# nguyenduchuyiu/marl-delivery

Hardware: AMD Instinct MI355X
Metric: agent-steps/sec (whole node), map1 5-agent 4096 envs, 1/2/4/8 MI355X (higher is better)
Workload: dtype int32+fp64

## Files before the change

marl-delivery_amd/csrc/mdl_device.hpp:

```cpp
#pragma once
#include <hip/hip_runtime.h>
#include <stdint.h>

#if !defined(MDL_PROFILING_BUILD) && \
    (defined(MDL_EXP_NOWAIT) || defined(MDL_EXP_NOTUPLES) || defined(MDL_EXP_NOLDS) || defined(MDL_ABLATE) || \
     defined(MDL_STAMPS))
#error "MDL_EXP_NOWAIT / MDL_EXP_NOTUPLES / MDL_EXP_NOLDS / MDL_ABLATE / MDL_STAMPS need -DMDL_PROFILING_BUILD"
#endif
#ifndef MDL_ABLATE
#define MDL_ABLATE 0
#endif

namespace mdl {

constexpr int WAVE = 64;
constexpr int MT_N = 624;
constexpr int MT_M = 397;
constexpr int MAX_MAPS = 8;
constexpr int PKG_PAD = 256;

enum : int { ST_NONE = 0, ST_WAITING = 1, ST_IN_TRANSIT = 2, ST_DELIVERED = 3 };
enum : int { MV_S = 0, MV_L = 1, MV_R = 2, MV_U = 3, MV_D = 4, MV_OTHER = 5 };
enum : int { SH_PICK = 0, SH_ONTIME, SH_LATE, SH_CLOSER, SH_WPICK, SH_WDROP, SH_STUCK, SH_IDLE, SH_AWAY };

struct MapDesc {
    int H, W, nfree;
    int grid_off;
    int free_off;
    int rank_off;
    float inv_hw;
    int bits_off;
    int mvc_off;
};

struct __align__(16) EnvScalars {
    int32_t t;
    uint32_t ctr;
    double total;
};
enum : uint32_t { RT_MOVE = 1u, RT_ONTIME = 2u, RT_LATE = 4u };

enum : uint32_t { PS_STATUS = 3u, PS_PRESENT = 4u, PS_TRANSIT = 8u, PS_SURVIVOR = 16u, PS_FLAGS = 31u };
constexpr int PS_RANK_SHIFT = 5;

constexpr uint32_t ORD_EPISODE = 0x400u;

struct DevParams {
    int E, A, P, T;
    double move_cost, delivery_reward, delay_reward;
    double cost_sum[9];
    float shaping[9];
    int stale;
    int obsT, MO, MP, MR, MPs;
    int n_maps;
    int key32_dsh;
    MapDesc maps[MAX_MAPS];
    const uint8_t* grids;
    const uint8_t* movevalid;
    const uint8_t* movevalid_cell;
    const uint32_t* gridbits;
    const uint16_t* free_cells;
    const uint16_t* rank;
    const uint8_t* env_map;
    uint32_t* rob;
    uint64_t* pkg;
    uint16_t* pstate;
    EnvScalars* es;
    uint32_t* mt;
    int32_t* mt_pos;
    uint64_t* trk;
    double* ep_total;
    int32_t* ep_len;
    const double* obs_recip;
    int obs_plane_words;
    int obs_small;
    int key7_dsh;
    double cost_fold[65];
};

__host__ __device__ __forceinline__ uint32_t rob_pack(int cell, int carry, uint32_t valid_mask ) {
    return (uint32_t)cell | ((uint32_t)carry << 16) | ((valid_mask & 0x1eu) << 26);
}
__host__ __device__ __forceinline__ int rob_cell(uint32_t w) { return (int)(w & 0xffffu); }
__host__ __device__ __forceinline__ int rob_carry(uint32_t w) { return (int)((w >> 16) & 0x7ffu); }
__host__ __device__ __forceinline__ uint32_t rob_valid(uint32_t w) { return (w >> 26) & 0x1eu; }

__device__ __forceinline__ int lane_id() { return (int)(threadIdx.x & 63); }
__device__ __forceinline__ int wave_id() { return __builtin_amdgcn_readfirstlane((int)(threadIdx.x >> 6)); }

__device__ __forceinline__ int xcd_slot(int b, int nb) { return (b & 7) * (nb >> 3) + min(b & 7, nb & 7) + (b >> 3); }
__device__ __forceinline__ int xcd_block() {
    return xcd_slot((int)blockIdx.x, (int)gridDim.x);
}

__device__ __forceinline__ void wave_sync() {
    __builtin_amdgcn_fence(__ATOMIC_RELEASE, "wavefront");
    __builtin_amdgcn_wave_barrier();
    __builtin_amdgcn_fence(__ATOMIC_ACQUIRE, "wavefront");
}

__device__ __forceinline__ uint64_t ballot(bool p) { return __ballot(p); }

#define GLOBAL __attribute__((address_space(1)))
typedef unsigned int u32x4 __attribute__((ext_vector_type(4)));

template <class T>
__device__ __forceinline__ void pin(T& v) { asm volatile("" : "+s"(v)); }

__device__ __forceinline__ int rdl(int v, int j) { return __builtin_amdgcn_readlane(v, j); }
__device__ __forceinline__ float rdlf(float v, int j) {
    return __int_as_float(__builtin_amdgcn_readlane(__float_as_int(v), j));
}
__device__ __forceinline__ int uni(int v) { return __builtin_amdgcn_readfirstlane(v); }

__device__ __forceinline__ uint32_t lmask(bool b) {
    uint32_t x = b ? ~0u : 0u;
    asm("" : "+v"(x));
    return x;
}
__device__ __forceinline__ uint32_t vbit(uint64_t m, int lane) { return 0u - (uint32_t)((m >> lane) & 1ull); }
__device__ __forceinline__ float fmask(uint32_t m, float a) { return __uint_as_float(m & __float_as_uint(a)); }
__device__ __forceinline__ float fpick(uint32_t m, float a, float b) {
    return __uint_as_float((m & __float_as_uint(a)) | (~m & __float_as_uint(b)));
}
__device__ __forceinline__ int ipick(uint32_t m, int a, int b) { return (int)((m & (uint32_t)a) | (~m & (uint32_t)b)); }

__device__ __forceinline__ int popc64(uint64_t m) { return __popcll(m); }
__device__ __forceinline__ int ffs64(uint64_t m) { return __ffsll((long long)m) - 1; }
__device__ __forceinline__ uint64_t lanemask_lt() {
    int l = lane_id();
    return l == 0 ? 0ull : (~0ull >> (64 - l));
}

__device__ __forceinline__ uint32_t wave_min_u32(uint32_t v) {
    const int id = (int)0xffffffff;
    uint32_t t;
    t = (uint32_t)__builtin_amdgcn_update_dpp(id, (int)v, 0x111, 0xf, 0xf, false); v = t < v ? t : v;
    t = (uint32_t)__builtin_amdgcn_update_dpp(id, (int)v, 0x112, 0xf, 0xf, false); v = t < v ? t : v;
    t = (uint32_t)__builtin_amdgcn_update_dpp(id, (int)v, 0x114, 0xf, 0xf, false); v = t < v ? t : v;
    t = (uint32_t)__builtin_amdgcn_update_dpp(id, (int)v, 0x118, 0xf, 0xf, false); v = t < v ? t : v;
    t = (uint32_t)__builtin_amdgcn_update_dpp(id, (int)v, 0x142, 0xa, 0xf, false); v = t < v ? t : v;
    t = (uint32_t)__builtin_amdgcn_update_dpp(id, (int)v, 0x143, 0xc, 0xf, false); v = t < v ? t : v;
    return (uint32_t)__builtin_amdgcn_readlane((int)v, 63);
}

__device__ __forceinline__ void wave_min_u32x2(uint32_t u, uint32_t v, uint32_t& mu, uint32_t& mv) {
    const int id = (int)0xffffffff;
    uint32_t a, b;
#define MDL_MIN2(ctl, rm)                                                                  \
    a = (uint32_t)__builtin_amdgcn_update_dpp(id, (int)u, ctl, rm, 0xf, false);            \
    b = (uint32_t)__builtin_amdgcn_update_dpp(id, (int)v, ctl, rm, 0xf, false);            \
    u = a < u ? a : u;                                                                     \
    v = b < v ? b : v;
    MDL_MIN2(0x111, 0xf)
    MDL_MIN2(0x112, 0xf)
    MDL_MIN2(0x114, 0xf)
    MDL_MIN2(0x118, 0xf)
    MDL_MIN2(0x142, 0xa)
    MDL_MIN2(0x143, 0xc)
#undef MDL_MIN2
    mu = (uint32_t)__builtin_amdgcn_readlane((int)u, 63);
    mv = (uint32_t)__builtin_amdgcn_readlane((int)v, 63);
}

__device__ __forceinline__ int wave_min8_lane(int a) { return ((a >> 1) << 4) | ((a & 1) << 3); }
__device__ __forceinline__ uint32_t wave_min8_u32(const uint32_t (&k)[8]) {
    uint32_t m[4], n[2];
#pragma unroll
    for (int i = 0; i < 4; i++) {
        const auto r = __builtin_amdgcn_permlane32_swap(k[i], k[i + 4], false, false);
        m[i] = r[0] < r[1] ? r[0] : r[1];
    }
#pragma unroll
    for (int i = 0; i < 2; i++) {
        const auto r = __builtin_amdgcn_permlane16_swap(m[i], m[i + 2], false, false);
        n[i] = r[0] < r[1] ? r[0] : r[1];
    }
    const bool hi = (lane_id() & 8) != 0;
    const uint32_t keep = hi ? n[1] : n[0], send = hi ? n[0] : n[1];
    const int id = (int)0xffffffff;
    uint32_t t = (uint32_t)__builtin_amdgcn_update_dpp(id, (int)send, 0x128, 0xf, 0xf, false);
    uint32_t v = t < keep ? t : keep;
    t = (uint32_t)__builtin_amdgcn_update_dpp(id, (int)v, 0x141, 0xf, 0xf, false);
    v = t < v ? t : v;
    t = (uint32_t)__builtin_amdgcn_update_dpp(id, (int)v, 0x4E, 0xf, 0xf, false);
    v = t < v ? t : v;
    t = (uint32_t)__builtin_amdgcn_update_dpp(id, (int)v, 0xB1, 0xf, 0xf, false);
    return t < v ? t : v;
}

__device__ __forceinline__ float qdiv_r(int a, double y) { return (float)((double)a * y); }

__device__ __forceinline__ float qdiv(int a, int b) { return (float)a / (float)b; }

__device__ __forceinline__ int fdivi(int i, int d, float inv) {
    int q = (int)((float)i * inv);
    int r = i - q * d;
    if (r < 0) q -= 1;
    else if (r >= d) q += 1;
    return q;
}

__device__ __forceinline__ int cell_r(int pc) { return pc & 255; }
__device__ __forceinline__ int cell_c(int pc) { return (pc >> 8) & 255; }
__device__ __forceinline__ int manhattan(int a, int b) {
    return abs(cell_r(a) - cell_r(b)) + abs(cell_c(a) - cell_c(b));
}
__device__ __forceinline__ int manhattan_sad(int a, int b) {
    return (int)__builtin_amdgcn_sad_u8((uint32_t)a, (uint32_t)b, 0u);
}

__device__ __forceinline__ int pk_start(uint64_t v) { return (int)(v & 0xffff); }
__device__ __forceinline__ int pk_target(uint64_t v) { return (int)((v >> 16) & 0xffff); }
__device__ __forceinline__ int pk_st(uint64_t v) { return (int)((v >> 32) & 0xffff); }
__device__ __forceinline__ int pk_dl(uint64_t v) { return (int)(v >> 48); }
__device__ __forceinline__ uint64_t pk_make(int start, int target, int st, int dl) {
    return (uint64_t)(uint32_t)start | ((uint64_t)(uint32_t)target << 16) | ((uint64_t)(uint32_t)st << 32) |
           ((uint64_t)(uint32_t)dl << 48);
}

__device__ __forceinline__ void decode_action(int a, int fmt, int& mv, int& op) {
    if (fmt == 0) {
        const int q = a / 5;
        const int m = a - 5 * q;
        mv = (0x30214 >> (4 * m)) & 0xf;
        op = q >= 3 ? 0 : q;
    } else {
        mv = a & 7;
        op = (a >> 3) & 3;
        if (mv > MV_OTHER) mv = MV_OTHER;
    }
}

__device__ inline void mt_twist(uint32_t* key) {
    const int lane = lane_id();
    for (int base = 0; base < MT_N; base += WAVE) {
        const int i = base + lane;
        uint32_t v = 0;
        if (i < MT_N) {
            const uint32_t y = (key[i] & 0x80000000u) | (key[i + 1 == MT_N ? 0 : i + 1] & 0x7fffffffu);
            const int k = i + MT_M < MT_N ? i + MT_M : i + MT_M - MT_N;
            v = key[k] ^ (y >> 1) ^ ((y & 1u) ? 0x9908b0dfu : 0u);
        }
        wave_sync();
        if (i < MT_N) key[i] = v;
        wave_sync();
    }
}

struct MTState {
    uint32_t* key;
    int pos;
};

__device__ inline uint32_t mt_next32(MTState& s) {
    if (s.pos == MT_N) {
        mt_twist(s.key);
        s.pos = 0;
    }
    uint32_t y = s.key[s.pos];
    s.pos++;
    y ^= (y >> 11);
    y ^= (y << 7) & 0x9d2c5680u;
    y ^= (y << 15) & 0xefc60000u;
    y ^= (y >> 18);
    return (uint32_t)uni((int)y);
}

__device__ inline int randint(MTState& s, int lo, int hi) {
    const uint32_t rng = (uint32_t)(hi - 1 - lo);
    if (rng == 0) return lo;
    uint32_t mask = rng;
    mask |= mask >> 1; mask |= mask >> 2; mask |= mask >> 4; mask |= mask >> 8; mask |= mask >> 16;
    uint32_t v;
    do {
        v = mt_next32(s) & mask;
    } while (v > rng);
    return lo + (int)v;
}

struct ResetOut {
    int robot_cell;
};

__device__ inline int reset_env(MTState& mt, const DevParams& p, const MapDesc& md, uint64_t* pk, uint8_t* pst,
                                uint64_t* scratch, uint16_t* taken) {
    const int lane = lane_id();
    const int A = p.A, P = p.P;
    const uint16_t* fl = p.free_cells + md.free_off;
    const int F = md.nfree;
    int my_cell = 0;
    int ntk = 0;
    for (int i = 0; i < A; i++) {
        const int k = randint(mt, 0, F - i);
        int idx = k;
        for (int q = 0; q < ntk; q++) {
            const int tq = taken[q];
            if (tq <= idx) idx++;
            else break;
        }
        if (lane == 0) {
            int q = ntk;
            while (q > 0 && taken[q - 1] > idx) {
                taken[q] = taken[q - 1];
                q--;
            }
            taken[q] = (uint16_t)idx;
        }
        ntk++;
        wave_sync();
        if (lane == i) my_cell = fl[idx];
    }
    const int N = md.H;
    const int lim = A < 20 ? A : 20;
    for (int i = 0; i < P; i++) {
        const int s_idx = randint(mt, 0, F);
        int t_idx;
        do {
            t_idx = randint(mt, 0, F);
        } while (t_idx == s_idx);
        const int to_dl = 10 + randint(mt, N / 2, 3 * N);
        const int st = (i <= lim) ? 0 : randint(mt, 1, p.T);
        if (lane == 0) scratch[i] = pk_make(s_idx, t_idx, st, st + to_dl);
    }
    wave_sync();
    for (int j = lane; j < P; j += WAVE) {
        const uint64_t v = scratch[j];
        scratch[j] = pk_make(fl[pk_start(v)], fl[pk_target(v)], pk_st(v), pk_dl(v));
    }
    wave_sync();
    for (int j0 = 0; j0 < P; j0 += WAVE) {
        const int j = j0 + lane;
        uint64_t v = 0;
        int sj = 0, rank = 0;
        if (j < P) {
            v = scratch[j];
            sj = pk_st(v);
        }
        for (int i = 0; i < P; i++) {
            const int si = pk_st(scratch[i]);
            rank += (si < sj) || (si == sj && i < j);
        }
        if (j < P) {
            pk[rank] = v;
        }
    }
    wave_sync();
    for (int j = lane; j < P; j += WAVE) pst[j] = pk_st(pk[j]) == 0 ? ST_WAITING : ST_NONE;
    wave_sync();
    return my_cell;
}

struct TrkFresh {
    static constexpr bool kIdIndexed = true;
    const uint64_t* pk;
    const uint8_t* ps;
    int n;
    __device__ int count() const { return n; }
    __device__ bool present(int j) const { const int s = ps[j] & PS_STATUS; return s == ST_WAITING || s == ST_IN_TRANSIT; }
    __device__ bool in_transit(int j) const { return (ps[j] & PS_STATUS) == ST_IN_TRANSIT; }
    __device__ uint64_t data(int j) const { return pk[j]; }
    __device__ int id(int j) const { return j + 1; }
    __device__ uint32_t order(int j) const { return (uint32_t)j; }
    __device__ int slot_of(int id) const { return (id >= 1 && id <= n && present(id - 1)) ? id - 1 : -1; }
};

struct TrkStale {
    static constexpr bool kIdIndexed = true;
    const uint8_t* ps;
    const uint64_t* td;
    const uint32_t* tq;
    int n;
    __device__ int count() const { return n; }
    __device__ bool present(int j) const { return (ps[j] & PS_PRESENT) != 0; }
    __device__ bool in_transit(int j) const { return (ps[j] & PS_TRANSIT) != 0; }
    __device__ uint64_t data(int j) const { return td[j]; }
    __device__ int id(int j) const { return j + 1; }
    __device__ uint32_t order(int j) const { return tq[j]; }
    __device__ int slot_of(int id) const { return (id >= 1 && id <= n && present(id - 1)) ? id - 1 : -1; }
};

struct TrkView {
    static constexpr bool kIdIndexed = false;
    const int32_t* ids;
    const uint8_t* flag;
    const uint64_t* pk;
    int n;
    __device__ int count() const { return n; }
    __device__ bool present(int j) const { return flag[j] & 1; }
    __device__ bool in_transit(int j) const { return (flag[j] & 2) != 0; }
    __device__ uint64_t data(int j) const { return pk[j]; }
    __device__ int id(int j) const { return ids[j]; }
    __device__ uint32_t order(int j) const { return (uint32_t)j; }
    __device__ int slot_of(int id) const {
        for (int j = 0; j < n; j++)
            if (ids[j] == id) return j;
        return -1;
    }
};

template <class Trk>
__device__ inline float shaped_agent(const Trk& trk, const float* C, bool active, int prev_cell, int prev_carry,
                                     int cur_cell, int cur_carry, int mv, int op, int t_prev, int t_cur) {
    float s = 0.0f;
    const int pslot = (active && prev_carry != 0) ? trk.slot_of(prev_carry) : -1;
    if (prev_carry == 0 && cur_carry != 0) {
        s = s + C[SH_PICK];
    } else if (prev_carry != 0 && cur_carry == 0) {
        if (pslot >= 0) {
            const uint64_t d = trk.data(pslot);
            if (cur_cell == pk_target(d)) s = s + ((t_cur <= pk_dl(d)) ? C[SH_ONTIME] : C[SH_LATE]);
        }
    }
    const bool moved = prev_cell != cur_cell;
    const bool need_can = active && op == 1 && prev_carry == 0 && cur_carry == 0;
    const bool need_near = active && moved && !(prev_carry != 0 && pslot >= 0);
    const bool need_idle = active && !moved && mv == MV_S && prev_carry == 0;
    bool can = false, idle = false;
    int best_d = 0x7fffffff;
    uint32_t best_o = 0xffffffffu;
    int best_cell = -1;
    if (__ballot(need_can || need_near || need_idle)) {
        const int n = trk.count();
        for (int j = 0; j < n; j++) {
            if (!trk.present(j) || trk.in_transit(j)) continue;
            const uint64_t d = trk.data(j);
            if (pk_st(d) > t_prev) continue;
            const int sc = pk_start(d);
            can |= sc == cur_cell;
            const int md = manhattan(prev_cell, sc);
            idle |= md <= 3;
            const uint32_t o = trk.order(j);
            if (md < best_d || (md == best_d && o < best_o)) {
                best_d = md;
                best_o = o;
                best_cell = sc;
            }
        }
    }
    if (op == 1) {
        if (prev_carry != 0) s = s + C[SH_WPICK];
        else if (cur_carry == 0 && !can) s = s + C[SH_WPICK];
    } else if (op == 2) {
        if (prev_carry == 0) s = s + C[SH_WDROP];
        else if (cur_carry != 0 && pslot >= 0 && cur_cell != pk_target(trk.data(pslot))) s = s + C[SH_WDROP];
    }
    if (mv != MV_S && !moved) s = s + C[SH_STUCK];
    int target = -1;
    if (prev_carry != 0 && pslot >= 0) target = pk_target(trk.data(pslot));
    else target = best_cell;
    if (target >= 0 && moved) {
        const int db = manhattan(prev_cell, target), da = manhattan(cur_cell, target);
        if (da < db) s = s + C[SH_CLOSER];
        else if (da > db) s = s + C[SH_AWAY];
    }
    if (!moved && mv == MV_S && prev_carry == 0 && idle) s = s + C[SH_IDLE];
    return active ? s : 0.0f;
}

template <int AU>
__device__ inline float np_sum_lanes8(float v, int n) {
    static_assert(AU >= 1 && AU <= 8, "np_sum_lanes8: 1 <= AU <= 8");
    float x[8];
#pragma unroll
    for (int i = 0; i < 8; i++) x[i] = i < AU ? rdlf(v, i) : 0.0f;
    float res;
    if (AU == 8 && n == 8) {
        res = ((x[0] + x[1]) + (x[2] + x[3])) + ((x[4] + x[5]) + (x[6] + x[7]));
    } else {
        res = 0.0f;
#pragma unroll
        for (int i = 0; i < (AU < 7 ? AU : 7); i++) res = res + x[i];
    }
    return 0.0f + res;
}

__device__ inline float np_sum_lanes(float v, int n) {
    float res;
    if (n < 8) {
        res = 0.0f;
        for (int i = 0; i < n; i++) res = res + rdlf(v, i);
    } else {
        float r0 = rdlf(v, 0), r1 = rdlf(v, 1), r2 = rdlf(v, 2), r3 = rdlf(v, 3);
        float r4 = rdlf(v, 4), r5 = rdlf(v, 5), r6 = rdlf(v, 6), r7 = rdlf(v, 7);
        int i;
        for (i = 8; i < n - (n % 8); i += 8) {
            r0 = r0 + rdlf(v, i + 0); r1 = r1 + rdlf(v, i + 1); r2 = r2 + rdlf(v, i + 2); r3 = r3 + rdlf(v, i + 3);
            r4 = r4 + rdlf(v, i + 4); r5 = r5 + rdlf(v, i + 5); r6 = r6 + rdlf(v, i + 6); r7 = r7 + rdlf(v, i + 7);
        }
        res = ((r0 + r1) + (r2 + r3)) + ((r4 + r5) + (r6 + r7));
        for (; i < n; i++) res = res + rdlf(v, i);
    }
    return 0.0f + res;
}

template <int AU>
__device__ inline float np_sum_lanes_dpp(float v) {
    static_assert(AU >= 1 && AU <= 7, "np_sum_lanes_dpp: 1 <= AU <= 7");
    float t = v;
#pragma unroll
    for (int i = 1; i < AU; i++) {
        const float prev = __int_as_float(__builtin_amdgcn_update_dpp(0, __float_as_int(t), 0x111, 0xf, 0xf, true));
        t = v + prev;
    }
    return rdlf(t, AU - 1);
}

template <int CTL>
__device__ __forceinline__ float dppf(float x) {
    return __int_as_float(__builtin_amdgcn_update_dpp(0, __float_as_int(x), CTL, 0xf, 0xf, true));
}
__device__ inline float np_sum16_dpp(float v) {
    const float r = v + dppf<0x128>(v);
    const float s = r + dppf<0xB1>(r);
    const float c = s + dppf<0x4E>(s);
    const float d = c + dppf<0x124>(c);
    return 0.0f + rdlf(d, 0);
}

template <int AU>
__device__ inline float np_sum_step(float v, int n) {
    if constexpr (AU > 0 && AU <= 7) return np_sum_lanes_dpp<AU>(v);
    else if constexpr (AU == 16) return np_sum16_dpp(v);
    else if constexpr (AU == 8) return np_sum_lanes8<AU>(v, n);
    else return np_sum_lanes(v, n);
}

}
```

marl-delivery_amd/csrc/mdl_kernels.hip:

```cpp
#include <cstring>
#include <type_traits>

#include "mdl_kernels.hpp"
#include "mdl_features.hpp"
#include "mdl_obs_small.hpp"
#include "mdl_altfeat.hpp"


namespace mdl {

#ifdef MDL_STAMPS
__device__ uint64_t g_stamps[65536 * 16];
#define STAMP(k)                                      \
    do {                                              \
        __builtin_amdgcn_sched_barrier(0);            \
        stamp_[k] = __builtin_amdgcn_s_memtime();     \
        __builtin_amdgcn_sched_barrier(0);            \
    } while (0)
#else
#define STAMP(k) \
    do {         \
    } while (0)
#endif

__host__ __device__ inline int stage_floats(int A, int na, int MO, int MPc, int MR, int MPsc) {
    const int dc = actor_compact_dim(A, MO, MPc);
    const int a = actor_group(na, dc) * dc, cr = critic_compact_dim(A, MR, MPsc);
    return a > cr ? a : cr;
}

struct ResetLds {
    uint64_t* pk;
    uint64_t* scratch;
    uint32_t* mt;
    uint16_t* taken;
    uint8_t* pst;
};

__host__ __device__ constexpr size_t reset_lds_bytes(int P) {
    return align16(8 * (size_t)P) * 2 + align16(4 * MT_N) + align16(2 * 64) + align16((size_t)P);
}

__device__ inline ResetLds reset_carve(unsigned char* b, int P) {
    ResetLds L;
    size_t o = 0;
    L.pk = (uint64_t*)(b + o); o += align16(8 * (size_t)P);
    L.scratch = (uint64_t*)(b + o); o += align16(8 * (size_t)P);
    L.mt = (uint32_t*)(b + o); o += align16(4 * MT_N);
    L.taken = (uint16_t*)(b + o); o += align16(2 * 64);
    L.pst = b + o;
    return L;
}

__device__ inline void load_mt(const DevParams& p, int e, uint32_t* key) {
    const uint32_t* g = p.mt + (size_t)e * MT_N;
    for (int i = lane_id(); i < MT_N; i += WAVE) key[i] = g[i];
    wave_sync();
}

__device__ inline void store_mt(const DevParams& p, int e, const uint32_t* key, int pos) {
    uint32_t* g = p.mt + (size_t)e * MT_N;
    for (int i = lane_id(); i < MT_N; i += WAVE) g[i] = key[i];
    if (lane_id() == 0) p.mt_pos[e] = pos;
}

__device__ inline int do_reset(const DevParams& p, int e, const MapDesc& md, ResetLds& L, bool seeded_in_lds) {
    if (!seeded_in_lds) load_mt(p, e, L.mt);
    MTState ms{L.mt, seeded_in_lds ? MT_N : p.mt_pos[e]};
    const int cell = reset_env(ms, p, md, L.pk, L.pst, L.scratch, L.taken);
    store_mt(p, e, L.mt, ms.pos);
    return cell;
}

template <int NCH, int AU = 0>
__device__ inline void tracker_update_regs(uint32_t (&ps)[NCH], uint64_t (&td)[NCH], bool (&dirty)[NCH],
                                           const uint64_t (&pk)[NCH], int P, int A, int carry, int t) {
    const int lane = lane_id();
#pragma unroll
    for (int c = 0; c < NCH; c++) {
        const int j = c * WAVE + lane;
        const bool ins = (j < P) & (pk_st(pk[c]) == t) & !(ps[c] & PS_PRESENT);
        ps[c] = ins ? ((ps[c] & PS_STATUS) | PS_PRESENT) : ps[c];
        td[c] = ins ? pk[c] : td[c];
        dirty[c] = dirty[c] || ins;
    }
#pragma unroll
    for (int c = 0; c < NCH; c++) {
        const int id = c * WAVE + lane + 1;
        bool carried = false;
        if constexpr (AU > 0) {
            uint32_t ci[AU], mn = 0xffffffffu;
#pragma unroll
            for (int i = 0; i < AU; i++) ci[i] = (uint32_t)rdl(carry, i);
            __builtin_amdgcn_sched_barrier(0);
#pragma unroll
            for (int i = 0; i < AU; i++) mn = min(mn, ci[i] ^ (uint32_t)id);
            carried = mn == 0u;
        } else {
            for (int i = 0; i < A; i++) carried |= rdl(carry, i) == id;
        }
        const uint32_t upd = carried ? (ps[c] | PS_TRANSIT) : (ps[c] & PS_TRANSIT) ? (ps[c] & PS_STATUS) : ps[c];
        ps[c] = (ps[c] & PS_PRESENT) ? upd : ps[c];
    }
}

template <int NCH>
__device__ inline void tracker_update_bits(uint32_t (&ps)[NCH], uint64_t (&td)[NCH], bool (&dirty)[NCH],
                                           const uint64_t (&pk)[NCH], int P, int t, uint32_t carried_bits) {
    const int lane = lane_id();
#pragma unroll
    for (int c = 0; c < NCH; c++) {
        const int j = c * WAVE + lane;
        const bool ins = (j < P) & (pk_st(pk[c]) == t) & !(ps[c] & PS_PRESENT);
        ps[c] = ins ? ((ps[c] & PS_STATUS) | PS_PRESENT) : ps[c];
        td[c] = ins ? pk[c] : td[c];
        dirty[c] = dirty[c] || ins;
        const bool carried = (carried_bits >> c) & 1u;
        const uint32_t upd = carried ? (ps[c] | PS_TRANSIT) : (ps[c] & PS_TRANSIT) ? (ps[c] & PS_STATUS) : ps[c];
        ps[c] = (ps[c] & PS_PRESENT) ? upd : ps[c];
    }
}

template <int NCH>
__device__ inline void survivors_at_reset(uint32_t (&ps)[NCH], uint32_t (&tq)[NCH], int P) {
    const int lane = lane_id();
    uint32_t rk[NCH];
#pragma unroll
    for (int c = 0; c < NCH; c++) rk[c] = 0;
#pragma unroll
    for (int c2 = 0; c2 < NCH; c2++) {
        uint64_t m = ballot(c2 * WAVE + lane < P && (ps[c2] & PS_PRESENT));
        while (m) {
            const uint32_t ki = (uint32_t)rdl((int)tq[c2], ffs64(m));
            m &= m - 1;
#pragma unroll
            for (int c = 0; c < NCH; c++) rk[c] += ki < tq[c] ? 1u : 0u;
        }
    }
#pragma unroll
    for (int c = 0; c < NCH; c++) {
        if (c * WAVE + lane < P && (ps[c] & PS_PRESENT)) {
            tq[c] = rk[c];
            ps[c] = (ps[c] & PS_FLAGS) | PS_SURVIVOR | (rk[c] << PS_RANK_SHIFT);
        } else {
            ps[c] &= PS_STATUS;
        }
    }
}

__global__ __launch_bounds__(256) void k_seed(DevParams p, const uint32_t* __restrict__ seeds, int wpb,
                                              int lds_stride) {
    extern __shared__ __align__(16) unsigned char smem[];
    const int wave = wave_id();
    const int lane = lane_id();
    const int e = blockIdx.x * wpb + wave;
    if (wave >= wpb || e >= p.E) return;
    ResetLds L = reset_carve(smem + (size_t)wave * lds_stride, p.P);
    const MapDesc md = p.maps[p.env_map ? p.env_map[e] : 0];
    if (lane == 0) {
        uint32_t s = seeds[e];
        for (int i = 0; i < MT_N; i++) {
            L.mt[i] = s;
            s = 1812433253u * (s ^ (s >> 30)) + (uint32_t)(i + 1);
        }
    }
    wave_sync();
    const int cell = do_reset(p, e, md, L, true);
    if (lane < p.A)
        p.rob[(size_t)e * p.A + lane] = rob_pack(cell, 0, p.movevalid[md.grid_off + cell_r(cell) * md.W + cell_c(cell)]);
    for (int j = lane; j < p.P; j += WAVE) {
        const size_t g = (size_t)e * p.P + j;
        p.pkg[g] = L.pk[j];
        p.pstate[g] = L.pst[j];
    }
    if (lane == 0) {
        EnvScalars s;
        s.t = 0;
        s.ctr = 0;
        s.total = 0.0;
        p.es[e] = s;
        p.ep_total[e] = 0.0;
        p.ep_len[e] = 0;
    }
}

template <int NCH>
__global__ __launch_bounds__(256) void k_reset(DevParams p, const int* __restrict__ env_ids, int n, int wpb,
                                               int lds_stride) {
    extern __shared__ __align__(16) unsigned char smem[];
    const int wave = wave_id();
    const int lane = lane_id();
    const int w = xcd_block() * wpb + wave;
    if (wave >= wpb || w >= n) return;
    const int e = env_ids ? env_ids[w] : w;
    if ((unsigned)e >= (unsigned)p.E) return;
    const int A = p.A, P = p.P;
    ResetLds L = reset_carve(smem + (size_t)wave * lds_stride, P);
    const MapDesc md = p.maps[p.env_map ? p.env_map[e] : 0];
    uint32_t ps[NCH], tq[NCH];
#pragma unroll
    for (int c = 0; c < NCH; c++) {
        const int j = c * WAVE + lane;
        ps[c] = j < P ? p.pstate[(size_t)e * P + j] : 0u;
        tq[c] = (p.stale && (ps[c] & PS_SURVIVOR)) ? ps[c] >> PS_RANK_SHIFT : ORD_EPISODE + (uint32_t)j;
    }
    const int cell = do_reset(p, e, md, L, false);
    uint64_t pk[NCH], td[NCH];
    bool dirty[NCH];
    if (p.stale) survivors_at_reset<NCH>(ps, tq, P);
#pragma unroll
    for (int c = 0; c < NCH; c++) {
        const int j = c * WAVE + lane;
        pk[c] = j < P ? L.pk[j] : 0;
        ps[c] = (j < P ? L.pst[j] : 0u) | (p.stale ? (ps[c] & ~PS_STATUS) : 0u);
        td[c] = pk[c];
        dirty[c] = false;
    }
    if (p.stale) tracker_update_regs<NCH>(ps, td, dirty, pk, P, A, 0, 0);
    if (lane < A)
        p.rob[(size_t)e * A + lane] = rob_pack(cell, 0, p.movevalid[md.grid_off + cell_r(cell) * md.W + cell_c(cell)]);
#pragma unroll
    for (int c = 0; c < NCH; c++) {
        const int j = c * WAVE + lane;
        if (j < P) {
            const size_t g = (size_t)e * P + j;
            p.pkg[g] = pk[c];
            p.pstate[g] = (uint16_t)ps[c];
            if (dirty[c]) p.trk[g] = td[c];
        }
    }
    if (lane == 0) {
        EnvScalars s;
        s.t = 0;
        s.ctr = 0;
        s.total = 0.0;
        p.es[e] = s;
    }
}

__global__ __launch_bounds__(256) void k_tracker_clear(DevParams p, const int* __restrict__ env_ids, int n) {
    const int wave = wave_id();
    const int w = blockIdx.x * 4 + wave;
    if (w >= n) return;
    const int e = env_ids ? env_ids[w] : w;
    if ((unsigned)e >= (unsigned)p.E) return;
    for (int j = lane_id(); j < p.P; j += WAVE) {
        const size_t g = (size_t)e * p.P + j;
        p.pstate[g] &= (uint16_t)PS_STATUS;
    }
    if (lane_id() == 0) p.es[e].ctr = 0;
}

#define MDL_STEP_LB 256
template <int NCH, bool FUSED>
constexpr int step_wpe() { return (NCH <= 2 && !FUSED) ? 8 : 1; }
#define MDL_STEP_ATTR(NCH, FUSED) __attribute__((amdgpu_waves_per_eu(step_wpe<NCH, FUSED>())))
struct StepArgs {
    DevParams p;
    const uint8_t* actions;
    const int* env_ids;
    double* r_out;
    float* sh_out;
    uint8_t* done_out;
    int fmt, n, auto_reset, wpb, lds_stride, K;
};
typedef __attribute__((address_space(4))) const StepArgs* KargPtr;
static_assert(sizeof(StepArgs) + 256 <= 4096, "the step's kernel arguments stay inside the 4 KiB kernarg segment");

struct StepKarg {
    const uint32_t* rob;
    const uint64_t* pkg;
    const uint16_t* pst;
    const u32x4* es;
    const uint64_t* trk;
    const uint8_t* act;
    uint32_t ap, nw;
    StepArgs args;
};
constexpr uint32_t NW_IDS = 1u << 29, NW_MAP = 1u << 30;
constexpr uint32_t NW_SMALLMAP = 1u << 31;
constexpr int AP_NB_SHIFT = 18;
inline uint32_t pack_ap(int A, int P, int nblocks) {
    const uint32_t nb = nblocks < (1 << (32 - AP_NB_SHIFT)) ? (uint32_t)nblocks : 0u;
    return (uint32_t)A | ((uint32_t)P << 7) | (nb << AP_NB_SHIFT);
}

struct ObsArgs {
    float* amap;
    float* avec;
    float* cmap;
    float* cvec;
};

struct EpiArgs {
    uint8_t* active;
    uint8_t* filled;
};
typedef __attribute__((address_space(4))) const EpiArgs* EpiKargPtr;
constexpr size_t EPI_KARG_OFF = sizeof(StepArgs) + sizeof(ObsArgs);
static_assert(sizeof(StepArgs) % 8 == 0 && sizeof(ObsArgs) % 8 == 0, "EpiArgs starts where ObsArgs ends");

__device__ __forceinline__ void publish_tail(const Publish& pb) {
    __atomic_thread_fence(__ATOMIC_RELEASE);
    if (!pb.ctr) {
        if (lane_id() == 0) __hip_atomic_store(pb.seq, pb.value, __ATOMIC_RELAXED, __HIP_MEMORY_SCOPE_SYSTEM);
        return;
    }
    if (lane_id() == 0) {
        const unsigned waves = pb.expect ? pb.expect : gridDim.x * (blockDim.x / WAVE);
        if (atomicAdd(pb.ctr, 1u) - pb.base == waves - 1u) {
            __atomic_thread_fence(__ATOMIC_ACQ_REL);
            __hip_atomic_store(pb.seq, pb.value, __ATOMIC_RELEASE, __HIP_MEMORY_SCOPE_SYSTEM);
        }
    }
}

constexpr int MAIL_INLINE_CODES = 256;
struct MailArgs {
    MailRows m;
    Publish pb;
    uint8_t codes[MAIL_INLINE_CODES];
};

#include "mdl_step_common.hpp"

__host__ __device__ constexpr uint64_t move_lt_lanes(int k) {
    uint64_t m = 0;
    for (int l = 0; l < 64; l++)
        if (((l >> 4) << 2) + k < (l & 15)) m |= 1ull << l;
    return m;
}

template <bool STALE, int NCH, bool FUSED, int AU, bool OBS, bool MAIL = false, bool EPI = false>
__device__ __forceinline__ void step_body(const uint32_t* __restrict__ rob_pre, const uint64_t* __restrict__ pkg_pre,
                                          const uint16_t* __restrict__ pst_pre, const u32x4* __restrict__ es_pre,
                                          const uint64_t* __restrict__ trk_pre, const uint8_t* __restrict__ act_pre,
                                          uint32_t ap, uint32_t nw, const StepArgs& args, const ObsArgs& oa,
                                          const MailArgs* ma = nullptr) {
    static_assert(!OBS || (NCH == 1 && !FUSED && AU > 0 && AU <= 8), "fused observations: P <= 64, A <= 8");
    static_assert(!EPI || (OBS && !MAIL), "the episode form is the fused step + observation launch's");
    extern __shared__ __align__(16) unsigned char smem[];
    const DevParams& p = args.p;
#ifdef MDL_STAMPS
    uint64_t stamp_[16];
#endif
    STAMP(0);
    const int A = (int)(ap & 0x7fu), P = (int)((ap >> 7) & 0x7ffu);
    const int n_ = (int)(nw & 0xffffffu), wpb_ = (int)((nw >> 24) & 31u);
    GLOBAL const uint32_t* robp = (GLOBAL const uint32_t*)rob_pre;
    GLOBAL const uint64_t* pkgp = (GLOBAL const uint64_t*)pkg_pre;
    GLOBAL const uint16_t* pstp = (GLOBAL const uint16_t*)pst_pre;
    GLOBAL const u32x4* esp = (GLOBAL const u32x4*)es_pre;
    GLOBAL const uint64_t* trkp = (GLOBAL const uint64_t*)trk_pre;
    GLOBAL const uint8_t* actp = (GLOBAL const uint8_t*)act_pre;
    STAMP(1);

    const int wave = wave_id();
    const int lane = lane_id();
    const int nbp = (int)(ap >> AP_NB_SHIFT);
    const int w = (nbp ? xcd_slot((int)blockIdx.x, nbp) : (int)blockIdx.x) * wpb_ + wave;
    if (wave >= wpb_ || w >= n_) return;
    int e = w;
    if (nw & NW_IDS) {
        e = uni(((GLOBAL const int*)args.env_ids)[w]);
        if ((unsigned)e >= (unsigned)args.p.E) return;
    }
    if constexpr (EPI) {
        KargPtr ka = (KargPtr)((__attribute__((address_space(4))) const char*)
                                   __builtin_amdgcn_kernarg_segment_ptr() + offsetof(StepKarg, args));
        asm volatile("" : "+s"(ka));
        EpiKargPtr ke = (EpiKargPtr)((__attribute__((address_space(4))) const char*)ka + EPI_KARG_OFF);
        if (!uni((int)((GLOBAL const uint8_t*)ke->active)[w])) {
            if (lane == 0) {
// ... 1640 lines not shown
```

Baseline: 4.950 billion.

## Vectorize Mersenne Twister draws across the wave with ballot-based rejection sampling

Replaces the serial per-draw MT19937 consumer in environment reset with a 64-wide window. All lanes temper one word each, and rejection sampling picks the next accepted draw with a ballot and find-first-set, so the output stream stays the same. Agent cell de-duplication becomes a ballot/popcount fixed-point loop instead of a lane-0 sorted insert, and global MT state loads are batched into registers before being written to LDS. It aims to cut the serial latency of resets, at the cost of more complex bookkeeping for the window position.

```diff
diff --git a/marl-delivery_amd/csrc/mdl_device.hpp b/marl-delivery_amd/csrc/mdl_device.hpp
--- a/marl-delivery_amd/csrc/mdl_device.hpp
+++ b/marl-delivery_amd/csrc/mdl_device.hpp
@@ -234,6 +234,7 @@
 
 __device__ inline void mt_twist(uint32_t* key) {
     const int lane = lane_id();
+#pragma unroll 1
     for (int base = 0; base < MT_N; base += WAVE) {
         const int i = base + lane;
         uint32_t v = 0;
@@ -248,87 +249,111 @@
     }
 }
 
-struct MTState {
+struct MTWindow {
     uint32_t* key;
-    int pos;
-};
-
-__device__ inline uint32_t mt_next32(MTState& s) {
-    if (s.pos == MT_N) {
-        mt_twist(s.key);
-        s.pos = 0;
-    }
-    uint32_t y = s.key[s.pos];
-    s.pos++;
+    int base;
+    uint64_t rem;
+    uint32_t w;
+    __device__ int len() const { return min(WAVE, MT_N - base); }
+    __device__ int pos() const { return base + (rem ? ffs64(rem) : WAVE); }
+};
+__device__ inline void mt_fill(MTWindow& s) {
+    uint32_t y = lane_id() < s.len() ? s.key[s.base + lane_id()] : 0u;
     y ^= (y >> 11);
     y ^= (y << 7) & 0x9d2c5680u;
     y ^= (y << 15) & 0xefc60000u;
     y ^= (y >> 18);
-    return (uint32_t)uni((int)y);
-}
-
-__device__ inline int randint(MTState& s, int lo, int hi) {
+    s.w = y;
+    s.rem = ~0ull;
+}
+__device__ inline MTWindow mt_window(uint32_t* key, int pos) {
+    MTWindow s{key, pos, 0ull, 0u};
+    mt_fill(s);
+    return s;
+}
+__device__ inline void mt_refill(MTWindow& s) {
+    s.base += s.len();
+    if (s.base == MT_N) {
+        mt_twist(s.key);
+        s.base = 0;
+    }
+    mt_fill(s);
+}
+
+__device__ __forceinline__ uint32_t draw_mask(uint32_t rng) { return 0xffffffffu >> __clz((int)rng); }
+__device__ __forceinline__ uint64_t range_accept(const MTWindow& s, uint32_t rng) {
+    return __builtin_amdgcn_ballot_w64(lane_id() < s.len() && (s.w & draw_mask(rng)) <= rng);
+}
+
+__device__ __forceinline__ int window_take(MTWindow& s, uint64_t acc) {
+    const uint64_t m = acc & s.rem;
+    if (!m) return -1;
+    const int k = ffs64(m);
+    s.rem = ~1ull << k;
+    return k;
+}
+
+__device__ inline int randint(MTWindow& s, int lo, int hi) {
     const uint32_t rng = (uint32_t)(hi - 1 - lo);
     if (rng == 0) return lo;
-    uint32_t mask = rng;
-    mask |= mask >> 1; mask |= mask >> 2; mask |= mask >> 4; mask |= mask >> 8; mask |= mask >> 16;
-    uint32_t v;
-    do {
-        v = mt_next32(s) & mask;
-    } while (v > rng);
-    return lo + (int)v;
-}
-
-struct ResetOut {
-    int robot_cell;
-};
-
-__device__ inline int reset_env(MTState& mt, const DevParams& p, const MapDesc& md, uint64_t* pk, uint8_t* pst,
-                                uint64_t* scratch, uint16_t* taken) {
+    int k;
+    while ((k = window_take(s, range_accept(s, rng))) < 0) mt_refill(s);
+    return lo + (int)((uint32_t)rdl((int)s.w, k) & draw_mask(rng));
+}
+
+__device__ inline int reset_env(MTWindow& mt, const DevParams& p, const MapDesc& md, uint64_t* pk, uint8_t* pst,
+                                uint64_t* scratch, uint16_t* cells) {
     const int lane = lane_id();
     const int A = p.A, P = p.P;
     const uint16_t* fl = p.free_cells + md.free_off;
     const int F = md.nfree;
-    int my_cell = 0;
-    int ntk = 0;
-    for (int i = 0; i < A; i++) {
-        const int k = randint(mt, 0, F - i);
-        int idx = k;
-        for (int q = 0; q < ntk; q++) {
-            const int tq = taken[q];
-            if (tq <= idx) idx++;
-            else break;
-        }
-        if (lane == 0) {
-            int q = ntk;
-            while (q > 0 && taken[q - 1] > idx) {
-                taken[q] = taken[q - 1];
-                q--;
+    {
+        int tk = 0;
+#pragma unroll 1
+        for (int i = 0; i < A; i++) {
+            const int k = randint(mt, 0, F - i);
+            int idx = k;
+            for (;;) {
+                const int nx = k + popc64(__builtin_amdgcn_ballot_w64(lane < i && tk <= idx));
+                if (nx == idx) break;
+                idx = nx;
             }
-            taken[q] = (uint16_t)idx;
-        }
-        ntk++;
-        wave_sync();
-        if (lane == i) my_cell = fl[idx];
+            tk = lane == i ? idx : tk;
+        }
+        cells[lane] = fl[lane < A ? tk : 0];
     }
     const int N = md.H;
     const int lim = A < 20 ? A : 20;
+    const uint32_t rngF = (uint32_t)(F - 1);
+    uint64_t accF = range_accept(mt, rngF);
+    auto draw_cell = [&]() {
+        int k;
+        while ((k = window_take(mt, accF)) < 0) {
+            mt_refill(mt);
+            accF = range_accept(mt, rngF);
+        }
+        return (uint32_t)rdl((int)mt.w, k) & draw_mask(rngF);
+    };
+#pragma unroll 1
     for (int i = 0; i < P; i++) {
-        const int s_idx = randint(mt, 0, F);
-        int t_idx;
+        const uint32_t s_idx = draw_cell();
+        uint32_t t_idx;
         do {
-            t_idx = randint(mt, 0, F);
+            t_idx = draw_cell();
         } while (t_idx == s_idx);
         const int to_dl = 10 + randint(mt, N / 2, 3 * N);
         const int st = (i <= lim) ? 0 : randint(mt, 1, p.T);
-        if (lane == 0) scratch[i] = pk_make(s_idx, t_idx, st, st + to_dl);
+        accF = range_accept(mt, rngF);
+        scratch[i] = pk_make((int)s_idx, (int)t_idx, st, st + to_dl);
     }
     wave_sync();
+#pragma unroll 1
     for (int j = lane; j < P; j += WAVE) {
         const uint64_t v = scratch[j];
         scratch[j] = pk_make(fl[pk_start(v)], fl[pk_target(v)], pk_st(v), pk_dl(v));
     }
     wave_sync();
+#pragma unroll 1
     for (int j0 = 0; j0 < P; j0 += WAVE) {
         const int j = j0 + lane;
         uint64_t v = 0;
@@ -346,9 +371,10 @@
         }
     }
     wave_sync();
+#pragma unroll 1
     for (int j = lane; j < P; j += WAVE) pst[j] = pk_st(pk[j]) == 0 ? ST_WAITING : ST_NONE;
     wave_sync();
-    return my_cell;
+    return (int)cells[lane];
 }
 
 struct TrkFresh {
diff --git a/marl-delivery_amd/csrc/mdl_kernels.hip b/marl-delivery_amd/csrc/mdl_kernels.hip
--- a/marl-delivery_amd/csrc/mdl_kernels.hip
+++ b/marl-delivery_amd/csrc/mdl_kernels.hip
@@ -33,7 +33,7 @@
     uint64_t* pk;
     uint64_t* scratch;
     uint32_t* mt;
-    uint16_t* taken;
+    uint16_t* cells;
     uint8_t* pst;
 };
 
@@ -47,14 +47,26 @@
     L.pk = (uint64_t*)(b + o); o += align16(8 * (size_t)P);
     L.scratch = (uint64_t*)(b + o); o += align16(8 * (size_t)P);
     L.mt = (uint32_t*)(b + o); o += align16(4 * MT_N);
-    L.taken = (uint16_t*)(b + o); o += align16(2 * 64);
+    L.cells = (uint16_t*)(b + o); o += align16(2 * 64);
     L.pst = b + o;
     return L;
 }
 
 __device__ inline void load_mt(const DevParams& p, int e, uint32_t* key) {
     const uint32_t* g = p.mt + (size_t)e * MT_N;
-    for (int i = lane_id(); i < MT_N; i += WAVE) key[i] = g[i];
+    const int lane = lane_id();
+    constexpr int ROUNDS = (MT_N + WAVE - 1) / WAVE;
+    uint32_t v[ROUNDS];
+#pragma unroll
+    for (int k = 0; k < ROUNDS; k++) {
+        const int i = k * WAVE + lane;
+        v[k] = i < MT_N ? g[i] : 0u;
+    }
+#pragma unroll
+    for (int k = 0; k < ROUNDS; k++) {
+        const int i = k * WAVE + lane;
+        if (i < MT_N) key[i] = v[k];
+    }
     wave_sync();
 }
 
@@ -66,9 +78,9 @@
 
 __device__ inline int do_reset(const DevParams& p, int e, const MapDesc& md, ResetLds& L, bool seeded_in_lds) {
     if (!seeded_in_lds) load_mt(p, e, L.mt);
-    MTState ms{L.mt, seeded_in_lds ? MT_N : p.mt_pos[e]};
-    const int cell = reset_env(ms, p, md, L.pk, L.pst, L.scratch, L.taken);
-    store_mt(p, e, L.mt, ms.pos);
+    MTWindow ms = mt_window(L.mt, seeded_in_lds ? MT_N : p.mt_pos[e]);
+    const int cell = reset_env(ms, p, md, L.pk, L.pst, L.scratch, L.cells);
+    store_mt(p, e, L.mt, ms.pos());
     return cell;
 }
 
```

Result: no change. 4.985 billion, median of 6 (+0.7%).
